# ZhiHuangHn/vtkCloudPoint

Hardware: AMD Instinct MI355X
Metric: Mpoints/s DBSCAN+label @10M pts (higher is better)
Workload: dtype f64; 1 GPU; C4: 10000000-pt cloud (half uniform background, 200 Gaussian blobs), one monolithic DBImproved.dbscan, metric L1_2D, eps 0.1, minPts 10; mode=single, points_total=10000000, points_per_gpu=10000000, clusters=27380, resident_in_hbm=True

## Files before the change

vtkcloudpoint_amd/csrc/dbscan.hip:

```cpp
#include <string.h>

#include <cmath>
#include <cstdlib>
#include <cstring>
#include <limits>
#include <vector>

#include "bounds.hpp"
#include "dbscan_engine.hpp"
#include "grid_common.hpp"

using namespace vcpg;

namespace {

#ifndef VCP_UNR2
#define VCP_UNR2 4
#endif
#ifndef VCP_UNR3
#define VCP_UNR3 2
#endif
#ifndef VCP_UNRW
#define VCP_UNRW 4
#endif
// ... 49 lines not shown
  double q[3], r[3];
  load_exact<GD>(xs, p, q);
  load_exact<GD>(xs, j, r);
  return within<METRIC>(q, r, thr);
}

template <int GD>
struct RowOrder;
template <>
struct RowOrder<2> {
  static constexpr int at(int k) { return k; }
};
template <>
struct RowOrder<3> {
  static constexpr int at(int k) {
    constexpr int o[9] = {1, 3, 4, 5, 7, 0, 2, 6, 8};
    return o[k];
  }
};

template <int GD, bool OWN_FIRST = false, class F>
__device__ __forceinline__ void for_rows(const int* cc, const GridP& g, const CellTab& ct, F&& f) {
  constexpr int NR = GD == 3 ? 9 : 3;
  const int x0 = max(cc[0] - 1, 0), x1 = min(cc[0] + 1, g.D[0] - 1);
  uint32_t rs[NR], re[NR];
#pragma unroll
  for (int r = 0; r < NR; r++) {
    const int y = cc[1] + (r % 3) - 1;
    const int z = GD == 3 ? cc[2] + (r / 3) - 1 : 0;
    const bool ok = y >= 0 && y < g.D[1] && (GD != 3 || (z >= 0 && z < g.D[2]));
    const uint32_t base = ok ? cell_id<GD>(g, 0, y, z) : 0u;
    rs[r] = re[r] = 0u;
    if (ok) ct_range(ct, base + x0, base + x1 + 1, rs[r], re[r]);
  }
  for (int k = 0; k < NR; k++) {
    const int r = OWN_FIRST ? RowOrder<GD>::at(k) : k;
    if (rs[r] < re[r])
      if (!f(rs[r], re[r])) return;
  }
}

template <int GD>
__device__ __forceinline__ void row_bounds(const int* cc, const GridP& g, const CellTab& ct, uint32_t* rs, uint32_t* re) {
  constexpr int NR = GD == 3 ? 9 : 3;
  const int x0 = max(cc[0] - 1, 0), x1 = min(cc[0] + 1, g.D[0] - 1);
#pragma unroll
  for (int r = 0; r < NR; r++) {
    const int y = cc[1] + (r % 3) - 1;
    const int z = GD == 3 ? cc[2] + (r / 3) - 1 : 0;
    const bool ok = y >= 0 && y < g.D[1] && (GD != 3 || (z >= 0 && z < g.D[2]));
    const uint32_t base = ok ? cell_id<GD>(g, 0, y, z) : 0u;
    rs[r] = re[r] = 0u;
    if (ok) ct_range(ct, base + x0, base + x1 + 1, rs[r], re[r]);
  }
}

constexpr unsigned XCHUNK = 8;
constexpr unsigned LCHUNK = 1;
__device__ __forceinline__ int64_t xcd_block(unsigned nblocks) {
  const unsigned b = blockIdx.x;
  const unsigned per = nblocks / (8u * XCHUNK);
  if (b >= per * 8u * XCHUNK) return b;
  const unsigned x = b & 7u, i = b >> 3;
  return (int64_t)((i / per) * 8u + x) * per + (i % per);
}

struct WorkList {
  uint32_t* list;
  const uint32_t* scan;
  uint32_t perblk;
  uint32_t nblk;
};

__device__ __forceinline__ uint32_t wl_fetch(const WorkList& w) {
  const uint32_t total = w.scan[w.nblk] - w.scan[0];
  const uint32_t x = blockIdx.x & 7u, i = blockIdx.x >> 3;
  const uint32_t c = (i / w.perblk) * 8u + x;
  const uint32_t lo = (uint32_t)(((uint64_t)total * c) / (8u * LCHUNK));
  const uint32_t hi = (uint32_t)(((uint64_t)total * (c + 1u)) / (8u * LCHUNK));
  const uint32_t t = lo + (i % w.perblk) * TPB + threadIdx.x;
  if (t >= hi) return NONE;
  return w.list[t];
}

__device__ __forceinline__ void wl_count(bool isE, bool isB, uint32_t blk, uint32_t* __restrict__ cntE,
                                         uint32_t* __restrict__ cntB) {
  __shared__ unsigned wc[2][TPB / 64];
  const unsigned long long mE = __ballot(isE), mB = __ballot(isB);
  if ((threadIdx.x & 63) == 0) {
    wc[0][threadIdx.x >> 6] = (unsigned)__popcll(mE);
    wc[1][threadIdx.x >> 6] = (unsigned)__popcll(mB);
  }
  __syncthreads();
  if (threadIdx.x == 0) {
    unsigned a = 0, b = 0;
    for (int k = 0; k < TPB / 64; k++) {
      a += wc[0][k];
      b += wc[1][k];
    }
    cntE[blk] = a;
    cntB[blk] = b;
  }
}

__global__ __launch_bounds__(TPB) void k_wl_fill(const uint8_t* __restrict__ flags, CellTab ct, const uint32_t* __restrict__ scanE,
                                                const uint32_t* __restrict__ scanB, uint32_t* __restrict__ listE,
// ... 138 lines not shown
        if (jj != (uint32_t)p) lnb[(nrec++) * TPB + threadIdx.x] = jj;
      }
      if (cnt >= min_pts) return false;
    }
    return true;
  });
  if (cnt >= min_pts) nrec = min(nrec, no.core_cap);
  uint8_t fl = live && has_cls ? flags[p] : 0;
  bool isE = false, isB = false;
  if (!live) {
  } else if (cnt >= min_pts) {
    fl |= F_CORE;
    if (!(fl & F_CLASSED)) {
      fl |= F_EXPAND;
      isE = true;
    } else {
      isB = true;
    }
  } else {
    isB = cnt > 1;
  }
  if (isB) fl |= F_BCAND;
  if (live) {
    flags[p] = fl | (uint8_t)(nrec << 4);
    parent[p] = isE ? (uint32_t)p : NONE;
    if (isE) minord[p] = NONE;
  }
  nbr_flush(no, lnb, lnb + no.NB * TPB, nrec, blk, p, live);
  wl_count(isE, isB, (uint32_t)blk, blkE, blkB);
}

template <int GD>
struct CoreTile;
template <>
struct CoreTile<2> {
  static constexpr int NR = 3, CAP = 512;
  union {
    float2 pt[3][512 + 4];
    uint32_t lout[15 * TPB];
  };
  uint32_t lo[3], hi[3];
  __device__ __forceinline__ void put(int r, uint32_t k, const float* __restrict__ s32, uint32_t pos) {
    pt[r][k] = reinterpret_cast<const float2*>(s32)[pos];
  }
  __device__ __forceinline__ void get(int r, uint32_t k, float* c) const {
    const float2 v = pt[r][k];
    c[0] = v.x;
    c[1] = v.y;
  }
};

template <int GD>
__device__ __forceinline__ bool tile_bounds(CoreTile<GD>& t, bool live, const int* cc, const GridP& g,
                                            const CellTab& ct, uint32_t* rs, uint32_t* re) {
  constexpr int NR = CoreTile<GD>::NR;
  if (threadIdx.x < NR) {
    t.lo[threadIdx.x] = NONE;
    t.hi[threadIdx.x] = 0u;
  }
  if (live) {
    row_bounds<GD>(cc, g, ct, rs, re);
  } else {
#pragma unroll
    for (int r = 0; r < NR; r++) rs[r] = re[r] = 0u;
  }
  __syncthreads();
#pragma unroll
  for (int r = 0; r < NR; r++) {
    const unsigned long long m = __ballot(rs[r] < re[r]);
    if (m) {
      const int f = __ffsll((long long)m) - 1, l = 63 - __clzll((long long)m);
      const uint32_t a = (uint32_t)__builtin_amdgcn_readlane((int)rs[r], f);
      const uint32_t b = (uint32_t)__builtin_amdgcn_readlane((int)re[r], l);
      if ((threadIdx.x & 63) == 0) {
        atomicMin(&t.lo[r], a);
        atomicMax(&t.hi[r], b);
      }
    }
  }
  __syncthreads();
  bool fits = true;
#pragma unroll
  for (int r = 0; r < NR; r++) fits = fits && (t.hi[r] <= t.lo[r] || t.hi[r] - t.lo[r] <= (uint32_t)CoreTile<GD>::CAP);
  return fits;
}

template <int GD>
__device__ __forceinline__ void tile_load(CoreTile<GD>& t, const float* __restrict__ sorted32,
                                          int32_t (*tg)[CoreTile<GD>::CAP + 4] = nullptr,
                                          const int32_t* __restrict__ sgroup = nullptr) {
#pragma unroll
  for (int r = 0; r < CoreTile<GD>::NR; r++) {
    const uint32_t lo = t.lo[r], hi = t.hi[r];
    if (hi > lo)
      for (uint32_t k = threadIdx.x; k < hi - lo; k += TPB) {
        t.put(r, k, sorted32, lo + k);
        if (tg) tg[r][k] = sgroup[lo + k];
      }
  }
  __syncthreads();
}

template <int GD, int METRIC>
__device__ __forceinline__ void nbr_flush_masks(const NbrOut& no, uint32_t* lout, const uint32_t* hm, const uint32_t* rs,
                                                const uint32_t* re, bool rescan, int nrec, double thr, const ExactSrc& xs,
                                                int64_t blk, int64_t p, bool live,
                                                const int32_t* __restrict__ sgroup = nullptr) {
  if (no.NB == 0) return;
  constexpr int NR = CoreTile<GD>::NR;
  __shared__ uint32_t wtot[TPB / 64];
  const int lane = threadIdx.x & 63, w = threadIdx.x >> 6;
  uint32_t pre, wsum;
  wave_prefix_small((uint32_t)nrec, pre, wsum);
  if (lane == 0) wtot[w] = wsum;
  __syncthreads();
  uint32_t total = 0;
  for (int k = 0; k < TPB / 64; k++) {
    if (k < w) pre += wtot[k];
    total += wtot[k];
  }
  if (live) no.off[p] = (uint16_t)pre;
  int k = 0;
  if (rescan) {
    double q[3];
    load_exact<GD>(xs, (uint32_t)p, q);
#pragma unroll
    for (int r = 0; r < NR; r++)
      for (uint32_t j = rs[r]; j < re[r] && k < nrec; j++) {
        double rr[3];
        load_exact<GD>(xs, j, rr);
        if (j != (uint32_t)p && within<METRIC>(q, rr, thr) && (!sgroup || sgroup[j] == sgroup[p])) lout[pre + (k++)] = j;
      }
  } else {
#pragma unroll
    for (int r = 0; r < NR; r++) {
      uint32_t m = hm[r];
      while (m != 0u && k < nrec) {
        const uint32_t pos = rs[r] + (uint32_t)(__ffs((int)m) - 1);
        m &= m - 1u;
        if (pos != (uint32_t)p) lout[pre + (k++)] = pos;
      }
    }
  }
  __syncthreads();
  uint32_t* dst = no.nbr + (size_t)blk * (size_t)(no.NB * TPB);
  for (uint32_t i = threadIdx.x; i < total; i += TPB) dst[i] = lout[i];
}

template <int GD, int METRIC, bool GROUPED = false>
__global__ __launch_bounds__(TPB) void k_core_lds(ExactSrc xs, GridP g, double thr, int min_pts,
                                                 CellTab ct, const int32_t* __restrict__ sgroup, uint8_t* __restrict__ flags,
                                                 uint32_t* __restrict__ parent, uint32_t* __restrict__ minord,
                                                 uint32_t* __restrict__ blkE, uint32_t* __restrict__ blkB, NbrOut no,
                                                 const float* __restrict__ sorted32, Screen sc, bool has_cls) {
  constexpr int NR = CoreTile<GD>::NR;
  constexpr int OWN = NR / 2;
  __shared__ CoreTile<GD> t;
  __shared__ int32_t tg[GROUPED ? NR : 1][CoreTile<GD>::CAP + 4];
  const uint32_t nin = *ct.nin;
  const int64_t blk = xcd_block(gridDim.x);
  int64_t p = blk * TPB + threadIdx.x;
  const bool live = p < nin;
  int cc[3] = {0, 0, 0};
  float qf[3] = {0.f, 0.f, 0.f};
  int32_t myg = 0;
  if (live) {
    load_pt32<GD>(sorted32, p, qf);
    cell_of32<GD>(qf, g, cc);
    if (GROUPED) myg = sgroup[p];
  }
  uint32_t rs[NR], re[NR];
  const bool fits = tile_bounds<GD>(t, live, cc, g, ct, rs, re);
  constexpr int UNR = 4;
  const uint32_t scLO = sc.lo < 0.0f ? 0u : __float_as_uint(sc.lo) + 1u;
  const uint32_t scS = __float_as_uint(sc.hi) + 1u - scLO;
  int cnt = 0;
  uint32_t hm[NR], ovf = 0u;
#pragma unroll
  for (int r = 0; r < NR; r++) hm[r] = 0u;
  if (fits) {
    if constexpr (GROUPED) tile_load<GD>(t, sorted32, tg, sgroup);
    else tile_load<GD>(t, sorted32);
    if (live) {
#pragma unroll
      for (int k = 0; k < NR; k++) {
        const int r = RowOrder<GD>::at(k);
        if (cnt >= min_pts || rs[r] >= re[r]) continue;
        const uint32_t lo = t.lo[r];
        const uint32_t e = re[r] - lo, a = rs[r] - lo;
        for (uint32_t j = a; j < e; j += UNR) {
          float c[UNR][3];
#pragma unroll
          for (int u = 0; u < UNR; u++) t.get(r, j + u, c[u]);
          uint32_t w[UNR], nib = 0;
#pragma unroll
          for (int u = UNR - 1; u >= 0; u--) {
            w[u] = __float_as_uint(value32<METRIC>(qf, c[u])) - scLO;
            if (GROUPED) w[u] = tg[r][j + u] == myg ? w[u] : scS;
            nib = __builtin_amdgcn_alignbit(nib, w[u] - scS, 31);
          }
          nib &= 0xFu >> (4u - min(e - j, 4u));
          if (min(min(w[0], w[1]), min(w[2], w[3])) < scS) {
            double q[3];
            load_exact<GD>(xs, (uint32_t)p, q);
#pragma unroll
            for (int u = 0; u < UNR; u++)
              if (((nib >> u) & 1u) && w[u] < scS) {
                double rr[3];
                load_exact<GD>(xs, lo + j + u, rr);
                if (!within<METRIC>(q, rr, thr)) nib &= ~(1u << u);
              }
          }
          cnt += __popc(nib);
          const uint32_t sh = j - a;
          const uint32_t first32 = (uint32_t)((int32_t)(sh - 32u) >> 31);
          hm[r] |= (nib << (sh & 31u)) & first32;
          ovf |= nib & ~first32;
          if (cnt >= min_pts) break;
        }
      }
    }
  } else if (live) {
#pragma unroll
    for (int k = 0; k < NR; k++) {
      const int r = RowOrder<GD>::at(k);
      if (cnt >= min_pts) continue;
      for (uint32_t j = rs[r]; j < re[r]; j += UNR) {
        float rr[UNR][3];
#pragma unroll
        for (int u = 0; u < UNR; u++) load_pt32<GD>(sorted32, min(j + u, re[r] - 1), rr[u]);
        uint32_t nib = 0;
#pragma unroll
        for (int u = 0; u < UNR; u++)
          nib |= ((j + u < re[r]) && (!GROUPED || sgroup[j + u] == myg) &&
                  within_scr<GD, METRIC>(qf, rr[u], sc, xs, (uint32_t)p, j + u, thr)) ? (1u << u) : 0u;
        cnt += __popc(nib);
        const uint32_t sh = j - rs[r];
        hm[r] |= sh < 32u ? nib << sh : 0u;
        ovf |= sh < 32u ? 0u : nib;
        if (cnt >= min_pts) break;
      }
    }
  }
  const bool rescan = live && no.NB > 0 && ovf != 0u && cnt < min_pts;
  int nrec = 0;
  if (live && no.NB > 0) {
    if (rescan) {
      nrec = max(cnt - 1, 0);
    } else {
#pragma unroll
      for (int r = 0; r < NR; r++) nrec += __popc(hm[r]);
      const uint32_t sb = (uint32_t)p - rs[OWN];
      if (rs[OWN] < re[OWN] && sb < 32u && ((hm[OWN] >> sb) & 1u)) nrec--;
    }
    nrec = min(nrec, cnt >= min_pts ? no.core_cap : no.NB);
  }
  uint8_t fl = live && has_cls ? flags[p] : 0;
  bool isE = false, isB = false;
  if (!live) {
  } else if (cnt >= min_pts) {
    fl |= F_CORE;
    if (!(fl & F_CLASSED)) {
      fl |= F_EXPAND;
      isE = true;
    } else {
      isB = true;
    }
  } else {
    isB = cnt > 1;
  }
  if (isB) fl |= F_BCAND;
  if (live) {
    flags[p] = fl | (uint8_t)(nrec << 4);
    parent[p] = isE ? (uint32_t)p : NONE;
    if (isE) minord[p] = NONE;
  }
  nbr_flush_masks<GD, METRIC>(no, t.lout, hm, rs, re, rescan, nrec, thr, xs, blk, p, live, GROUPED ? sgroup : nullptr);
  wl_count(isE, isB, (uint32_t)blk, blkE, blkB);
}

__device__ __forceinline__ uint32_t ld_parent(const uint32_t* parent, uint32_t x) {
  return __hip_atomic_load(&parent[x], __ATOMIC_RELAXED, __HIP_MEMORY_SCOPE_AGENT);
}

__device__ __forceinline__ uint32_t ld_parent_cached(const uint32_t* parent, uint32_t x) {
  return __hip_atomic_load(&parent[x], __ATOMIC_RELAXED, __HIP_MEMORY_SCOPE_WAVEFRONT);
}

__device__ __forceinline__ uint32_t uf_root(uint32_t* parent, uint32_t x) {
  uint32_t p = ld_parent_cached(parent, x);
  while (p != x) {
    const uint32_t gp = ld_parent_cached(parent, p);
    if (gp == p) return p;
    __hip_atomic_store(&parent[x], gp, __ATOMIC_RELAXED, __HIP_MEMORY_SCOPE_WAVEFRONT);
    x = gp;
    p = ld_parent_cached(parent, x);
  }
  return x;
}
// ... 608 lines not shown
double l2_threshold(double eps) {
  if (std::isinf(eps)) return eps;
  double t = eps * eps;
  if (std::isinf(t)) t = std::numeric_limits<double>::max();
  while (std::sqrt(t) > eps) t = std::nextafter(t, 0.0);
  for (;;) {
    double u = std::nextafter(t, std::numeric_limits<double>::infinity());
    if (std::isinf(u) || std::sqrt(u) > eps) break;
    t = u;
  }
  return t;
}

Screen screen_bounds(int metric, int gd, double thr, double E) {
  Screen sc;
  sc.lo = -1.0f;
  sc.hi = INFINITY;
  if (!(thr >= 0.0) || !std::isfinite(E)) return sc;
  if ((thr > 0.0 && thr < 1e-30) || E > 1e18) return sc;
  const double u = 5.9604644775390625e-08;
  const double alpha = 2.0 * u * E * (1.0 + 2.0 * u);
  double err;
  bool lo_ok = true;
  if (metric == VCP_L1_2D) {
    err = 2.0 * alpha * (1.0 + u) + 2.0 * u * (1.0 + u) * thr;
  } else {
    err = 2.0 * alpha * std::sqrt((double)gd * thr) * (1.0 + u) + (double)gd * alpha * alpha + 6.0 * u * (1.0 + u) * thr;
    lo_ok = std::sqrt(thr) > 4.0 * alpha * std::sqrt((double)gd);
  }
  err = err * 1.0625 + 1e-14 * thr + 1e-300;
  const double lo = thr - err, hi = thr + err;
  if (std::isfinite(hi)) {
    float h = (float)hi;
    if ((double)h < hi) h = std::nextafterf(h, INFINITY);
    sc.hi = h;
  }
  if (lo_ok && lo >= 0.0 && std::isfinite(lo)) {
    float l = (float)lo;
    if ((double)l > lo) l = std::nextafterf(l, -INFINITY);
    sc.lo = l;
  } else if (lo_ok && std::isinf(thr) && thr > 0) {
    sc.lo = 3.4028234663852886e38f;
  }
  return sc;
}

unsigned list_perblk(int64_t n) {
  const int64_t band = (n + 8 * LCHUNK - 1) / (8 * LCHUNK) + 1;
  return vcp_blocks(band, TPB);
}

struct Switches {
  int64_t cells_per_point;
  bool screen_off, lists_off, core_global;
  int core_cap, join_all;
};
const Switches& switches() {
  static const Switches sw = [] {
    Switches s;
    const char* e = getenv("VCP_CELL_BUDGET");
    const long v = e ? atol(e) : 32;
    s.cells_per_point = (int64_t)(v < 1 ? 1 : v > 4096 ? 4096 : v);
    s.screen_off = getenv("VCP_NO_SCREEN") != nullptr;
    s.lists_off = getenv("VCP_NO_LISTS") != nullptr;
    s.core_global = getenv("VCP_CORE_GLOBAL") != nullptr;
    s.core_cap = getenv("VCP_CORE_CAP") ? atoi(getenv("VCP_CORE_CAP")) : -1;
    s.join_all = getenv("VCP_JOIN_ALL") ? atoi(getenv("VCP_JOIN_ALL")) : -1;
    return s;
  }();
  return sw;
}

struct EnginePinned {
  double bounds[8];
  uint32_t unclassed;
  uint32_t n_comp;
  unsigned long long counters[CNT_WORDS];
};
static_assert(sizeof(EnginePinned) <= 1024, "the engine's region of vcp_ctx::pinned");
EnginePinned* engine_pinned(vcp_ctx* ctx) { return reinterpret_cast<EnginePinned*>(ctx->pinned); }

struct Call {
  const double* d_coords;
  int64_t n;
  int stride, metric;
  double eps;
  int min_pts;
  int32_t cf_in;
  const uint8_t* d_in_classed;
  int32_t* d_labels;
  uint8_t *d_is_core, *d_is_classed;
  int32_t* cf_out;
  int64_t* dist_evals;
  const DbscanExt* ext;
  int gd = 2;
  unsigned nb = 0;
  const int32_t* d_group = nullptr;
  const uint32_t* d_ord = nullptr;
  uint32_t* d_group_twice = nullptr;
  int G = 0, glo = 0, ghi = 0;
  bool slab = false;
  double* h = nullptr;
  bool all_finite = false;
  double thr = 0.0;
  GridP g;
  Screen sc{-1.0f, INFINITY};
  bool flags_set = false, part_out = false;
  ExactSrc xs{nullptr, nullptr, 0};
  NbrOut no{nullptr, nullptr, 0, 0};
};
void call_derive(Call& c) {
  const DbscanExt* ext = c.ext;
  const bool grouped = ext && ext->d_group;
  c.gd = c.metric == VCP_L2_3D ? 3 : 2;
  c.nb = vcp_blocks(c.n, TPB);
  c.d_group = grouped ? ext->d_group : nullptr;
  c.d_ord = ext ? ext->d_ord : nullptr;
  c.d_group_twice = grouped ? ext->d_group_twice : nullptr;
// ... 245 lines not shown
    return vcp_fail(ctx, VCP_ERR_UNSUPPORTED, "the cloud's extent overflows binary64 (coordinate - origin is infinite)");
  g.scale = 1.0;
  if (Emax > 1e30 || (Emax > 0.0 && Emax < 1e-20)) g.scale = std::ldexp(1.0, -std::ilogb(Emax));
  g.inv_h = std::isinf(cellw) ? 0.0 : 1.0 / (cellw * g.scale);
  g.ncells = (uint32_t)ncells;
  return VCP_OK;
}

int stage_grid_build(vcp_ctx* ctx, Call& c, const Workspace& ws) {
  GridBuildArgs ga;
  ga.d_coords = c.d_coords;
  ga.n = c.n;
  ga.stride = c.stride;
  ga.gd = c.gd;
  ga.g = c.g;
  ga.d_group = c.d_group;
  ga.glo = c.glo;
  ga.ghi = c.ghi;
  ga.d_ord = c.d_ord;
  ga.d_in_classed = c.d_in_classed;
  ga.ctwords = ws.ctwords;
  ga.ctdense = ws.ctdense;
  ga.ctcount = ws.ctcount;
  ga.sidx = c.d_ord ? ws.cellof : nullptr;
  ga.sorted32 = ws.sorted32;
  ga.sord = ws.sord;
  ga.sgroup = ws.sgroup;
  ga.flags = ws.flags;
  ga.pos = c.part_out ? nullptr : ws.pos;
  VCP_TRY(vcp_grid_build_partition(ctx, ga));
  c.xs = ExactSrc{c.d_coords, c.d_ord ? ws.cellof : ws.sord, c.stride};
  return VCP_OK;
}

template <int GD, int METRIC, bool GROUPED>
int stage_core(vcp_ctx* ctx, Call& c, const Workspace& ws, const Switches& sw) {
  hipStream_t st = ctx->stream;
  const int64_t n = c.n;
  const unsigned nb = c.nb;
  vcp_phase(ctx, "core_count");
  NbrOut& no = c.no;
  if (!sw.lists_off && !c.d_in_classed && !c.slab && c.min_pts >= 2 && c.min_pts <= 16) {
    no.NB = c.min_pts - 1;
    VCP_TRY(vcp_ensure(ctx, ctx->b_nbr, (size_t)no.NB * (size_t)nb * TPB * 4));
    VCP_TRY(vcp_ensure(ctx, ctx->b_nboff, (size_t)nb * TPB * 2));
    no.nbr = ctx->b_nbr.as<uint32_t>();
    no.off = ctx->b_nboff.as<uint16_t>();
    no.core_cap = (GD == 2 && (uint64_t)n < (uint64_t)c.g.ncells) ? std::min(no.NB, CORE_LIST) : no.NB;
    if (sw.core_cap >= 0) no.core_cap = std::min(no.NB, sw.core_cap);
  }
  const size_t lds_nb = (size_t)no.NB * TPB * 4;
  bool tiled = false;
  if constexpr (GD == 2) {
    if (!GROUPED || !sw.core_global) {
      VCP_LAUNCH(ctx, (k_core_lds<GD, METRIC, GROUPED>), dim3(nb), dim3(TPB), 0, st, c.xs, c.g, c.thr, c.min_pts, ws.ct,
                      ws.sgroup, ws.flags, ws.parent, ws.minord, ws.blkE, ws.blkB, no, ws.sorted32, c.sc, c.flags_set);
      tiled = true;
    }
  }
  if (!tiled)
    VCP_LAUNCH(ctx, (k_core<GD, METRIC, GROUPED>), dim3(nb), dim3(TPB), 2 * lds_nb, st, c.xs, c.g, c.thr, c.min_pts, ws.ct,
                    ws.sgroup, ws.flags, ws.parent, ws.minord, ws.blkE, ws.blkB, no, ws.sorted32, c.sc, c.flags_set);
  VCP_TRY(vcp_exclusive_scan_u32(ctx, ws.blkE, ws.blkE, 2 * ((int64_t)nb + 2), nullptr));
  VCP_LAUNCH(ctx, k_wl_fill, dim3(nb), dim3(TPB), 0, st, ws.flags, ws.ct, ws.blkE, ws.blkB, ws.wlE.list, ws.wlB.list,
                  ws.seedflag, ws.nw, ws.counters, c.d_group_twice, (uint32_t)(GROUPED ? c.G : 0));
  return VCP_OK;
}

template <int GD, int METRIC, bool GROUPED>
int stage_union(vcp_ctx* ctx, const Call& c, const Workspace& ws, const Switches& sw) {
  hipStream_t st = ctx->stream;
  const int64_t n = c.n;
  const unsigned nb = c.nb, nbl = ws.nbl;
  const GridP& g = c.g;
  const NbrOut& no = c.no;
  vcp_phase(ctx, "union");
  const bool pre = GD == 2 || no.NB > 0;
  if (no.NB > 0) {
    VCP_LAUNCH(ctx, k_union_init_list, dim3(nbl), dim3(TPB), 0, st, ws.flags, ws.parent, no, ws.wlE);
    const bool all = sw.join_all >= 0 ? sw.join_all != 0 : (uint64_t)n >= (uint64_t)g.ncells;
    if (all) VCP_LAUNCH(ctx, k_flatten0<2>, dim3(nbl), dim3(TPB), 0, st, ws.parent, ws.wlE, ws.flags, no);
    else VCP_LAUNCH(ctx, k_flatten0<1>, dim3(nbl), dim3(TPB), 0, st, ws.parent, ws.wlE, ws.flags, no);
    VCP_LAUNCH(ctx, k_flatten0<0>, dim3(nbl), dim3(TPB), 0, st, ws.parent, ws.wlE, ws.flags, no);
  } else if (GD == 2) {
    VCP_LAUNCH(ctx, (k_union_init<GD, METRIC, GROUPED>), dim3(nbl), dim3(TPB), 0, st, c.xs, g, c.thr, ws.ct, ws.sgroup,
                    ws.flags, ws.parent, ws.wlE, ws.sorted32, c.sc);
    VCP_LAUNCH(ctx, k_flatten0<0>, dim3(nbl), dim3(TPB), 0, st, ws.parent, ws.wlE, ws.flags, no);
  }
  const bool dense = pre && (uint64_t)n > (uint64_t)DENSE_PER_CELL * g.ncells;
  if (dense) {
    VCP_TRY(vcp_ensure(ctx, ctx->b_aux0, ((size_t)nb * (TPB / 64) + 2) * 4));
    uint32_t* chunkroot = ctx->b_aux0.as<uint32_t>();
    VCP_LAUNCH(ctx, k_chunkroot, dim3(nb), dim3(TPB), 0, st, ws.parent, ws.ct, chunkroot);
    VCP_LAUNCH(ctx, (k_union<GD, METRIC, GROUPED, true, true>), dim3(nbl), dim3(TPB), 0, st, c.xs, g, c.thr, ws.ct,
                    ws.sgroup, ws.parent, ws.wlE, ws.sorted32, c.sc, chunkroot);
  } else if (pre)
    VCP_LAUNCH(ctx, (k_union<GD, METRIC, GROUPED, true>), dim3(nbl), dim3(TPB), 0, st, c.xs, g, c.thr, ws.ct, ws.sgroup,
                    ws.parent, ws.wlE, ws.sorted32, c.sc);
  else
    VCP_LAUNCH(ctx, (k_union<GD, METRIC, GROUPED, false>), dim3(nbl), dim3(TPB), 0, st, c.xs, g, c.thr, ws.ct, ws.sgroup,
                    ws.parent, ws.wlE, ws.sorted32, c.sc);
  return VCP_OK;
}

int stage_slab_handoff(vcp_ctx* ctx, const Call& c, const Workspace& ws) {
  hipStream_t st = ctx->stream;
  const unsigned nb = c.nb;
// ... 374 lines not shown
```

vtkcloudpoint_amd/csrc/grid_common.hpp:

```cpp
#pragma once
#include "vcp_ctx.hpp"

namespace vcpg {

constexpr int TPB = 256;
constexpr uint8_t F_CORE = 1, F_CLASSED = 2, F_EXPAND = 4, F_BCAND = 8;
constexpr uint32_t NONE = 0xFFFFFFFFu;

constexpr int CNT_LONELY = 0, CNT_MISSING = 0, CNT_SEED_TOTAL = 2, CNT_GROUP_EVALS = 3;
constexpr int CNT_SPREAD = 32;
constexpr int CNT_UNCLASSED = 4, CNT_TWICE = CNT_UNCLASSED + CNT_SPREAD, CNT_WORDS = CNT_TWICE + CNT_SPREAD;

struct GridP {
  double mn[3];
  double inv_h;
  double scale;
  int D[3];
  uint32_t ncells;
};

template <int GD>
__device__ __forceinline__ uint32_t cell_id(const GridP& g, int cx, int cy, int cz) {
  uint32_t id = (uint32_t)cy * (uint32_t)g.D[0] + (uint32_t)cx;
  if (GD == 3) id += (uint32_t)cz * (uint32_t)g.D[0] * (uint32_t)g.D[1];
// ... 38 lines not shown
}

template <int GD>
__device__ __forceinline__ void load_in(const double* __restrict__ c, int64_t i, int stride, double* q) {
  if (GD == 2 && stride == 2) {
    double2 v = *reinterpret_cast<const double2*>(c + 2 * i);
    q[0] = v.x;
    q[1] = v.y;
  } else {
#pragma unroll
    for (int a = 0; a < GD; a++) q[a] = c[i * stride + a];
  }
}

template <int GD>
__device__ __forceinline__ uint32_t cell_of(const double* q, const GridP& g, int* cc) {
  cc[0] = cell_coord(q[0], g.mn[0], g.scale, g.inv_h, g.D[0]);
  cc[1] = cell_coord(q[1], g.mn[1], g.scale, g.inv_h, g.D[1]);
  cc[2] = 0;
  if (GD == 3) cc[2] = cell_coord(q[2], g.mn[2], g.scale, g.inv_h, g.D[2]);
  return cell_id<GD>(g, cc[0], cc[1], cc[2]);
}

template <int GD>
__device__ __forceinline__ uint32_t cell_of32(const float* qf, const GridP& g, int* cc) {
  cc[0] = cell_coord32(qf[0], g.inv_h, g.D[0]);
  cc[1] = cell_coord32(qf[1], g.inv_h, g.D[1]);
  cc[2] = 0;
  if (GD == 3) cc[2] = cell_coord32(qf[2], g.inv_h, g.D[2]);
  return cell_id<GD>(g, cc[0], cc[1], cc[2]);
}

struct CellTab {
  const uint4* words;
  const uint32_t* dense;
  const uint32_t* nin;
};

__device__ __forceinline__ uint32_t ct_start(const CellTab& t, uint32_t cell) {
  const uint4 w = t.words[cell >> 5];
  const uint32_t i = cell & 31u, below = (1u << i) - 1u;
  if ((w.x & w.y & below) == 0u) return w.z + (uint32_t)__popc(w.x & below) + 2u * (uint32_t)__popc(w.y & below);
  return t.dense[(size_t)w.w * 32u + i];
}
__device__ __forceinline__ uint32_t ct_from_word(const CellTab& t, const uint4 w, uint32_t cell) {
  const uint32_t i = cell & 31u, below = (1u << i) - 1u;
  if ((w.x & w.y & below) == 0u) return w.z + (uint32_t)__popc(w.x & below) + 2u * (uint32_t)__popc(w.y & below);
  return t.dense[(size_t)w.w * 32u + i];
}
__device__ __forceinline__ void ct_range(const CellTab& t, uint32_t c0, uint32_t c1, uint32_t& s, uint32_t& e) {
  const uint4 w0 = t.words[c0 >> 5];
  s = ct_from_word(t, w0, c0);
  e = (c1 >> 5) == (c0 >> 5) ? ct_from_word(t, w0, c1) : ct_start(t, c1);
}

struct Screen {
  float lo, hi;
};

template <int GD>
__device__ __forceinline__ void load_pt32(const float* __restrict__ c, int64_t i, float* q) {
  if (GD == 2) {
    const float2 v = *reinterpret_cast<const float2*>(c + 2 * i);
    q[0] = v.x;
    q[1] = v.y;
  } else {
    const float4 v = *reinterpret_cast<const float4*>(c + 4 * i);
    q[0] = v.x;
    q[1] = v.y;
    q[2] = v.z;
  }
}
template <int GD>
__device__ __forceinline__ void store_pt32(float* __restrict__ c, int64_t i, const double* q, const GridP& g) {
  if (GD == 2) {
    *reinterpret_cast<float2*>(c + 2 * i) = make_float2(rel32(q[0], g.mn[0], g.scale), rel32(q[1], g.mn[1], g.scale));
  } else {
    *reinterpret_cast<float4*>(c + 4 * i) =
        make_float4(rel32(q[0], g.mn[0], g.scale), rel32(q[1], g.mn[1], g.scale), rel32(q[2], g.mn[2], g.scale), 0.0f);
  }
}

struct ExactSrc {
  const double* base;
  const uint32_t* idx;
  int stride;
};
template <int GD>
__device__ __forceinline__ void load_exact(const ExactSrc& xs, uint32_t p, double* q) {
  const int64_t i = xs.idx ? (int64_t)xs.idx[p] : (int64_t)p;
  load_in<GD>(xs.base, i, xs.stride, q);
}

}

struct GridBuildArgs {
  const double* d_coords = nullptr;
  int64_t n = 0;
  int stride = 2, gd = 2;
  vcpg::GridP g;
  const int32_t* d_group = nullptr;
  int glo = 0, ghi = 0;
  const uint32_t* d_ord = nullptr;
  const uint8_t* d_in_classed = nullptr;
  uint4* ctwords = nullptr;
  uint32_t* ctdense = nullptr;
// ... 28 lines not shown
```

vtkcloudpoint_amd/csrc/gridbuild.hip:

```cpp
#include <algorithm>
#include <mutex>
#include <unordered_map>

#include "grid_common.hpp"

using namespace vcpg;

namespace {

constexpr int PT = 1024;
constexpr int PCH_MIN = 8192;
constexpr int FT = 1024;
constexpr uint32_t MAXB = 8192;
constexpr uint32_t wcap(int) { return 4096u; }
constexpr uint32_t QUEUE_FROM = 32;

typedef float4 Rec;

template <int GD>
__device__ __forceinline__ Rec rec_make(const float* qf, uint32_t idx, uint32_t cell) {
  return GD == 2 ? make_float4(qf[0], qf[1], __uint_as_float(idx), __uint_as_float(cell))
                 : make_float4(qf[0], qf[1], qf[2], __uint_as_float(idx));
}
template <int GD>
// ... 521 lines not shown
  const uint32_t nq = *qcount;
  for (uint32_t qi = blockIdx.x; qi < nq; qi += gridDim.x) {
    const uint2 q = queue[qi];
    const uint32_t b = q.x, w0 = q.y;
    uint32_t s, e;
    bucket_range(bstart, bstride, total, b, B, s, e);
    const uint32_t m = e - s;
    for (uint32_t j = s + threadIdx.x; j < e; j += FT) {
      const Rec r = rec[j];
      uint32_t i;
      const uint32_t p = ct_start(ct, rec_cell<GD>(r, g, i)) + rk[j] - s - w0;
      if (p < WCAP) stage_put<GD>(s32, sidx, p, r, i);
    }
    __syncthreads();
    fine_flush<GD, GROUPED>(s + w0, min(WCAP, m - w0), s32, sidx, ord, in_classed, group, sorted32, sord, sidx_out, sgroup,
                            flags, pos);
    __syncthreads();
  }
}

constexpr int OT = 1024, OPT = 16;
constexpr int OWT = 512;

template <int OWSH>
__global__ __launch_bounds__(OT) void k_out_scatter(const uint32_t* __restrict__ sord, const uint32_t* __restrict__ labk,
                                                   int64_t n, uint32_t OB, uint32_t* __restrict__ gcur,
                                                   uint2* __restrict__ rec) {
  extern __shared__ uint32_t h[];
  for (uint32_t k = threadIdx.x; k < OB; k += OT) h[k] = 0;
  __syncthreads();
  const int64_t first = (int64_t)blockIdx.x * (OT * OPT);
  uint32_t o[OPT], w[OPT], r[OPT];
#pragma unroll
  for (int k = 0; k < OPT; k++) {
    const int64_t p = first + (int64_t)k * OT + threadIdx.x;
    o[k] = NONE;
    if (p < n) {
      o[k] = sord[p];
      w[k] = labk[p];
      r[k] = atomicAdd(&h[o[k] >> OWSH], 1u);
    }
  }
  __syncthreads();
  for (uint32_t k = threadIdx.x; k < OB; k += OT) {
    const uint32_t c = h[k];
    if (c) h[k] = atomicAdd(&gcur[k], c);
  }
  __syncthreads();
#pragma unroll
  for (int k = 0; k < OPT; k++) {
    if (o[k] == NONE) continue;
    const uint32_t bk = o[k] >> OWSH;
    rec[((size_t)bk << OWSH) + h[bk] + r[k]] = make_uint2(o[k], w[k]);
  }
}

template <int OWSH>
__global__ __launch_bounds__(OWT) void k_out_write(const uint2* __restrict__ rec, int64_t n, bool have_in_classed,
                                                  int32_t cf_in, int32_t* __restrict__ labels,
                                                  uint8_t* __restrict__ is_core, uint8_t* __restrict__ is_classed,
                                                  unsigned long long* __restrict__ counters, uint32_t* __restrict__ gcur) {
  extern __shared__ __attribute__((aligned(16))) uint32_t sw[];
  if (threadIdx.x == 0) gcur[blockIdx.x] = 0u;
  const int64_t lo = (int64_t)blockIdx.x << OWSH;
  const uint32_t cnt = (uint32_t)min((int64_t)1 << OWSH, n - lo);
  unsigned unclassed = 0;
  for (uint32_t j = threadIdx.x; j < cnt; j += OWT) {
    const uint2 v = rec[lo + j];
    sw[v.x - (uint32_t)lo] = v.y;
    if (!(v.y & 2u)) unclassed++;
  }
  __syncthreads();
  auto lab_of = [&](uint32_t w) { return (w >> 2) ? cf_in + (int32_t)(w >> 2) : 0; };
  auto core_of = [](uint32_t w) { return (uint32_t)((w & 3u) == 1u); };
  auto cls_of = [](uint32_t w) { return (uint32_t)((w & 2u) != 0u || (w >> 2) != 0u); };
  const bool vec = (((uintptr_t)labels & 15u) | ((uintptr_t)is_core & 3u) | ((uintptr_t)is_classed & 3u)) == 0;
  const uint32_t c4 = vec ? cnt >> 2 : 0u;
  for (uint32_t j = threadIdx.x; j < c4; j += OWT) {
    const uint4 w = reinterpret_cast<const uint4*>(sw)[j];
    const int4 l = make_int4(lab_of(w.x), lab_of(w.y), lab_of(w.z), lab_of(w.w));
    if (have_in_classed) {
      if (l.x) labels[lo + 4 * j] = l.x;
      if (l.y) labels[lo + 4 * j + 1] = l.y;
      if (l.z) labels[lo + 4 * j + 2] = l.z;
      if (l.w) labels[lo + 4 * j + 3] = l.w;
    } else {
      reinterpret_cast<int4*>(labels + lo)[j] = l;
    }
    if (is_core)
      reinterpret_cast<uint32_t*>(is_core + lo)[j] = core_of(w.x) | core_of(w.y) << 8 | core_of(w.z) << 16 | core_of(w.w) << 24;
    if (is_classed)
      reinterpret_cast<uint32_t*>(is_classed + lo)[j] = cls_of(w.x) | cls_of(w.y) << 8 | cls_of(w.z) << 16 | cls_of(w.w) << 24;
  }
  for (uint32_t j = (c4 << 2) + threadIdx.x; j < cnt; j += OWT) {
    const uint32_t w = sw[j];
    const int32_t l = lab_of(w);
    if (!have_in_classed || l) labels[lo + j] = l;
    if (is_core) is_core[lo + j] = (uint8_t)core_of(w);
    if (is_classed) is_classed[lo + j] = (uint8_t)cls_of(w);
  }
  if (have_in_classed) {
    __shared__ unsigned wc[OWT / 64];
#pragma unroll
    for (int d = 32; d > 0; d >>= 1) unclassed += __shfl_down(unclassed, d, 64);
    if ((threadIdx.x & 63) == 0) wc[threadIdx.x >> 6] = unclassed;
    __syncthreads();
// ... 55 lines not shown
    VCP_TRY(vcp_ensure(ctx, ctx->b_bstart, ((size_t)pg.B + 2) * 4));
    VCP_LAUNCH(ctx, k_part_split<GD>, dim3(pg.NS), dim3(FT), 0, st, rec, ctx->b_rec2.as<Rec>(), counts, total, pg.nchunk,
                    pg.NS, pg.a, pg.csh, pg.B, a.g, ctx->b_bstart.as<uint32_t>());
    rec = ctx->b_rec2.as<Rec>();
    bstart = ctx->b_bstart.as<uint32_t>();
    bstride = 1;
  }
  vcp_phase(ctx, "part_fine");
  VCP_TRY(vcp_ensure(ctx, ctx->b_rank, (size_t)a.n * 4));
  VCP_TRY(vcp_ensure(ctx, ctx->b_bstate, (size_t)pg.B + 16));
  uint8_t* bstate = ctx->b_bstate.as<uint8_t>();
  VCP_LAUNCH(ctx, (k_part_fine_small<GD, GROUPED>), dim3(pg.B), dim3(FS), 0, st, rec, bstart, bstride, total, pg.B, pg.csh,
                  a.g, a.d_ord, a.d_in_classed, a.d_group, a.ctwords, a.ctdense, a.ctcount, bstate, a.sorted32, a.sord,
                  a.sidx, a.sgroup, a.flags, a.pos);
  VCP_LAUNCH(ctx, (k_part_fine<GD, GROUPED>), dim3(pg.B), dim3(FT), lds_f, st, rec, ctx->b_rank.as<uint32_t>(), bstart,
                  bstride, total, pg.B, pg.csh, a.g, a.d_ord, a.d_in_classed, a.d_group, a.ctwords, a.ctdense, a.ctcount,
                  a.sorted32, a.sord, a.sidx, a.sgroup, a.flags, a.pos, queue, qcount, bstate);
  {
    const size_t lds_w = (size_t)wcap(GD) * ((GD == 2 ? 8 : 16) + 4);
    VCP_TRY(allow_lds(ctx, k_part_fine_windows<GD, GROUPED>, lds_w));
    const unsigned gw = (unsigned)std::min<size_t>(768, (size_t)a.n / wcap(GD) + 1);
    const CellTab ct{a.ctwords, a.ctdense, a.ctcount + 1};
    VCP_LAUNCH(ctx, (k_part_fine_windows<GD, GROUPED>), dim3(gw), dim3(FT), lds_w, st, rec, ctx->b_rank.as<uint32_t>(),
                    bstart, bstride, total, pg.B, a.g, a.d_ord, a.d_in_classed, a.d_group, ct, a.sorted32,
                    a.sord, a.sidx, a.sgroup, a.flags, a.pos, queue, qcount);
  }
  return VCP_OK;
}

}

int vcp_grid_build_partition(vcp_ctx* ctx, const GridBuildArgs& a) {
  const bool grouped = a.d_group != nullptr;
  if (a.gd == 3) {
    if (grouped) return vcp_fail(ctx, VCP_ERR_ARG, "grouped calls are 2-D");
    return build<3, false>(ctx, a);
  }
  return grouped ? build<2, true>(ctx, a) : build<2, false>(ctx, a);
}

template <int OWSH>
static int output_partition(vcp_ctx* ctx, const GridOutputArgs& a) {
  hipStream_t st = ctx->stream;
  const uint32_t OB = (uint32_t)((a.n + (1 << OWSH) - 1) >> OWSH);
  const void* before = ctx->b_outcur.p;
  const size_t before_cap = ctx->b_outcur.cap;
  VCP_TRY(vcp_ensure(ctx, ctx->b_outcur, ((size_t)OB + 8) * 4));
  if (ctx->b_outcur.p != before || ctx->b_outcur.cap != before_cap)
    VCP_HIP(ctx, hipMemsetAsync(ctx->b_outcur.p, 0, ctx->b_outcur.cap, st));
  VCP_TRY(vcp_ensure(ctx, ctx->b_rec, (size_t)OB << (OWSH + 3)));
  uint32_t* gcur = ctx->b_outcur.as<uint32_t>();
  uint2* rec = ctx->b_rec.as<uint2>();
  VCP_TRY(allow_lds(ctx, k_out_write<OWSH>, (size_t)4 << OWSH));
  vcp_phase(ctx, "out_scatter");
  VCP_LAUNCH(ctx, k_out_scatter<OWSH>, dim3(vcp_blocks(a.n, OT * OPT)), dim3(OT), (size_t)OB * 4, st, a.sord, a.labk, a.n,
                  OB, gcur, rec);
  vcp_phase(ctx, "out_write");
  VCP_LAUNCH(ctx, k_out_write<OWSH>, dim3(OB), dim3(OWT), (size_t)4 << OWSH, st, rec, a.n, a.have_in_classed, a.cf_in,
                  a.labels, a.is_core, a.is_classed, a.counters, gcur);
  return VCP_OK;
}

int vcp_grid_output_partition(vcp_ctx* ctx, const GridOutputArgs& a) {
  if (a.n > ((int64_t)1 << 27)) return vcp_fail(ctx, VCP_ERR_TOO_LARGE, "more than 2^27 points: use the gather output");
  if (a.n >= ((int64_t)1 << 23)) return output_partition<15>(ctx, a);
  if (a.n >= ((int64_t)1 << 22)) return output_partition<14>(ctx, a);
  return output_partition<13>(ctx, a);
}
```

Measured before the change: 7079 Mpoints/s.

## Skip neighbor scans for isolated points via 5x5 cell-count bitplane prefilter

```diff
diff --git a/vtkcloudpoint_amd/csrc/dbscan.hip b/vtkcloudpoint_amd/csrc/dbscan.hip
--- a/vtkcloudpoint_amd/csrc/dbscan.hip
+++ b/vtkcloudpoint_amd/csrc/dbscan.hip
@@ -125,6 +125,33 @@
     const uint32_t base = ok ? cell_id<GD>(g, 0, y, z) : 0u;
     rs[r] = re[r] = 0u;
     if (ok) ct_range(ct, base + x0, base + x1 + 1, rs[r], re[r]);
+  }
+}
+
+template <int GD>
+__device__ __forceinline__ void row_words(const int* cc, const GridP& g, const CellTab& ct, uint4* w) {
+  static_assert(GD == 2, "three rows");
+  const int x0 = max(cc[0] - 1, 0);
+#pragma unroll
+  for (int r = 0; r < 3; r++) {
+    const int y = cc[1] + r - 1;
+    const bool ok = y >= 0 && y < g.D[1];
+    w[r] = ct.words[(cell_id<GD>(g, 0, ok ? y : cc[1], 0) + (uint32_t)x0) >> 5];
+  }
+}
+template <int GD>
+__device__ __forceinline__ void row_bounds_from(const int* cc, const GridP& g, const CellTab& ct, const uint4* w,
+                                                uint32_t* rs, uint32_t* re) {
+  const int x0 = max(cc[0] - 1, 0), x1 = min(cc[0] + 1, g.D[0] - 1);
+#pragma unroll
+  for (int r = 0; r < 3; r++) {
+    const int y = cc[1] + r - 1;
+    rs[r] = re[r] = 0u;
+    if (y >= 0 && y < g.D[1]) {
+      const uint32_t c0 = cell_id<GD>(g, 0, y, 0) + (uint32_t)x0, c1 = cell_id<GD>(g, 0, y, 0) + (uint32_t)x1 + 1u;
+      rs[r] = ct_from_word(ct, w[r], c0);
+      re[r] = (c1 >> 5) == (c0 >> 5) ? ct_from_word(ct, w[r], c1) : ct_start(ct, c1);
+    }
   }
 }
 
@@ -369,14 +396,19 @@
 
 template <int GD>
 __device__ __forceinline__ bool tile_bounds(CoreTile<GD>& t, bool live, const int* cc, const GridP& g,
-                                            const CellTab& ct, uint32_t* rs, uint32_t* re) {
+                                            const CellTab& ct, uint32_t* rs, uint32_t* re, const uint4* pre = nullptr) {
   constexpr int NR = CoreTile<GD>::NR;
   if (threadIdx.x < NR) {
     t.lo[threadIdx.x] = NONE;
     t.hi[threadIdx.x] = 0u;
   }
   if (live) {
-    row_bounds<GD>(cc, g, ct, rs, re);
+    if constexpr (GD == 2) {
+      if (pre) row_bounds_from<GD>(cc, g, ct, pre, rs, re);
+      else row_bounds<GD>(cc, g, ct, rs, re);
+    } else {
+      row_bounds<GD>(cc, g, ct, rs, re);
+    }
   } else {
 #pragma unroll
     for (int r = 0; r < NR; r++) rs[r] = re[r] = 0u;
@@ -464,7 +496,44 @@
   for (uint32_t i = threadIdx.x; i < total; i += TPB) dst[i] = lout[i];
 }
 
-template <int GD, int METRIC, bool GROUPED = false>
+__device__ __forceinline__ bool quiet_point(bool live, const int* cc, const GridP& g, const CellTab& ct, int min_pts) {
+  const int x0 = max(cc[0] - 2, 0), x1 = min(cc[0] + 2, g.D[0] - 1);
+  constexpr int DY[5] = {0, -1, 1, -2, 2};
+  uint2 w0[5], w1[5];
+  uint32_t c0[5], full[5];
+#pragma unroll
+  for (int k = 0; k < 5; k++) {
+    const int y = cc[1] + DY[k];
+    const bool ok = y >= 0 && y < g.D[1];
+    const uint32_t base = (uint32_t)(ok ? y : cc[1]) * (uint32_t)g.D[0];
+    c0[k] = base + (uint32_t)x0;
+    full[k] = ok ? (2u << (x1 - x0)) - 1u : 0u;
+    w0[k] = ct_planes(ct, c0[k]);
+    w1[k] = ct_planes(ct, base + (uint32_t)x1);
+  }
+  bool sat = false, cand = live;
+  int S = (int)ct_pop_planes(w0[0], w1[0], c0[0], full[0], sat);
+  cand = cand && S < min_pts;
+  if (__ballot(cand) == 0ull) return false;
+  S += (int)(ct_pop_planes(w0[1], w1[1], c0[1], full[1], sat) + ct_pop_planes(w0[2], w1[2], c0[2], full[2], sat));
+  cand = cand && S < min_pts;
+  if (__ballot(cand) == 0ull) return false;
+  S += (int)(ct_pop_planes(w0[3], w1[3], c0[3], full[3], sat) + ct_pop_planes(w0[4], w1[4], c0[4], full[4], sat));
+  cand = cand && S < min_pts;
+  if (cand && sat) {
+    S = 0;
+    for (int dy = -2; dy <= 2; dy++) {
+      const int y = cc[1] + dy;
+      if (y < 0 || y >= g.D[1]) continue;
+      const uint32_t base = (uint32_t)y * (uint32_t)g.D[0];
+      S += (int)ct_pop_exact(ct, base + (uint32_t)x0, base + (uint32_t)x1);
+    }
+    cand = S < min_pts;
+  }
+  return cand;
+}
+
+template <int GD, int METRIC, bool GROUPED = false, bool QUIET = false>
 __global__ __launch_bounds__(TPB) void k_core_lds(ExactSrc xs, GridP g, double thr, int min_pts,
                                                  CellTab ct, const int32_t* __restrict__ sgroup, uint8_t* __restrict__ flags,
                                                  uint32_t* __restrict__ parent, uint32_t* __restrict__ minord,
@@ -481,13 +550,43 @@
   int cc[3] = {0, 0, 0};
   float qf[3] = {0.f, 0.f, 0.f};
   int32_t myg = 0;
+  uint32_t cid = 0u;
   if (live) {
     load_pt32<GD>(sorted32, p, qf);
-    cell_of32<GD>(qf, g, cc);
+    cid = cell_of32<GD>(qf, g, cc);
     if (GROUPED) myg = sgroup[p];
   }
+  bool act = live;
   uint32_t rs[NR], re[NR];
-  const bool fits = tile_bounds<GD>(t, live, cc, g, ct, rs, re);
+  bool fits;
+  if constexpr (QUIET) {
+    const unsigned long long lm = __ballot(live);
+    bool sparse = false;
+    if (lm != 0ull) {
+      const uint32_t c_first = (uint32_t)__builtin_amdgcn_readlane((int)cid, __ffsll((long long)lm) - 1);
+      const uint32_t c_last = (uint32_t)__builtin_amdgcn_readlane((int)cid, 63 - __clzll((long long)lm));
+      sparse = c_last - c_first >= (uint32_t)__popcll(lm);
+    }
+    uint4 rw[3];
+    row_words<GD>(cc, g, ct, rw);
+    if (sparse) act = live && !quiet_point(live, cc, g, ct, min_pts);
+    fits = tile_bounds<GD>(t, act, cc, g, ct, rs, re, rw);
+  } else {
+    fits = tile_bounds<GD>(t, act, cc, g, ct, rs, re);
+  }
+  if constexpr (QUIET) {
+    bool none = true;
+#pragma unroll
+    for (int r = 0; r < NR; r++) none = none && t.hi[r] <= t.lo[r];
+    if (none) {
+      if (live) {
+        flags[p] = has_cls ? (uint8_t)(flags[p] & F_CLASSED) : (uint8_t)0;
+        parent[p] = NONE;
+      }
+      if (threadIdx.x == 0) blkE[blk] = blkB[blk] = 0u;
+      return;
+    }
+  }
   constexpr int UNR = 4;
   const uint32_t scLO = sc.lo < 0.0f ? 0u : __float_as_uint(sc.lo) + 1u;
   const uint32_t scS = __float_as_uint(sc.hi) + 1u - scLO;
@@ -498,7 +597,7 @@
   if (fits) {
     if constexpr (GROUPED) tile_load<GD>(t, sorted32, tg, sgroup);
     else tile_load<GD>(t, sorted32);
-    if (live) {
+    if (act) {
 #pragma unroll
       for (int k = 0; k < NR; k++) {
         const int r = RowOrder<GD>::at(k);
@@ -537,7 +636,7 @@
         }
       }
     }
-  } else if (live) {
+  } else if (act) {
 #pragma unroll
     for (int k = 0; k < NR; k++) {
       const int r = RowOrder<GD>::at(k);
@@ -559,9 +658,9 @@
       }
     }
   }
-  const bool rescan = live && no.NB > 0 && ovf != 0u && cnt < min_pts;
+  const bool rescan = act && no.NB > 0 && ovf != 0u && cnt < min_pts;
   int nrec = 0;
-  if (live && no.NB > 0) {
+  if (act && no.NB > 0) {
     if (rescan) {
       nrec = max(cnt - 1, 0);
     } else {
@@ -1276,7 +1375,7 @@
 
 struct Switches {
   int64_t cells_per_point;
-  bool screen_off, lists_off, core_global;
+  bool screen_off, lists_off, core_global, no_quiet;
   int core_cap, join_all;
 };
 const Switches& switches() {
@@ -1288,6 +1387,7 @@
     s.screen_off = getenv("VCP_NO_SCREEN") != nullptr;
     s.lists_off = getenv("VCP_NO_LISTS") != nullptr;
     s.core_global = getenv("VCP_CORE_GLOBAL") != nullptr;
+    s.no_quiet = getenv("VCP_NO_QUIET") != nullptr;
     s.core_cap = getenv("VCP_CORE_CAP") ? atoi(getenv("VCP_CORE_CAP")) : -1;
     s.join_all = getenv("VCP_JOIN_ALL") ? atoi(getenv("VCP_JOIN_ALL")) : -1;
     return s;
@@ -1639,7 +1739,15 @@
   const size_t lds_nb = (size_t)no.NB * TPB * 4;
   bool tiled = false;
   if constexpr (GD == 2) {
-    if (!GROUPED || !sw.core_global) {
+    const bool quiet = !GROUPED && !sw.no_quiet && !c.d_in_classed && !c.slab && c.min_pts >= 2 &&
+                       (uint64_t)n < (uint64_t)c.g.ncells;
+    if (quiet) {
+      if constexpr (!GROUPED)
+        VCP_LAUNCH(ctx, (k_core_lds<GD, METRIC, false, true>), dim3(nb), dim3(TPB), 0, st, c.xs, c.g, c.thr, c.min_pts,
+                        ws.ct, ws.sgroup, ws.flags, ws.parent, ws.minord, ws.blkE, ws.blkB, no, ws.sorted32, c.sc,
+                        c.flags_set);
+      tiled = true;
+    } else if (!GROUPED || !sw.core_global) {
       VCP_LAUNCH(ctx, (k_core_lds<GD, METRIC, GROUPED>), dim3(nb), dim3(TPB), 0, st, c.xs, c.g, c.thr, c.min_pts, ws.ct,
                       ws.sgroup, ws.flags, ws.parent, ws.minord, ws.blkE, ws.blkB, no, ws.sorted32, c.sc, c.flags_set);
       tiled = true;
diff --git a/vtkcloudpoint_amd/csrc/grid_common.hpp b/vtkcloudpoint_amd/csrc/grid_common.hpp
--- a/vtkcloudpoint_amd/csrc/grid_common.hpp
+++ b/vtkcloudpoint_amd/csrc/grid_common.hpp
@@ -114,6 +114,22 @@
   const uint4 w0 = t.words[c0 >> 5];
   s = ct_from_word(t, w0, c0);
   e = (c1 >> 5) == (c0 >> 5) ? ct_from_word(t, w0, c1) : ct_start(t, c1);
+}
+
+__device__ __forceinline__ uint2 ct_planes(const CellTab& t, uint32_t cell) {
+  return *reinterpret_cast<const uint2*>(&t.words[cell >> 5]);
+}
+__device__ __forceinline__ uint32_t ct_pop_planes(const uint2 w0, const uint2 w1, uint32_t c0, uint32_t full, bool& sat) {
+  const unsigned long long m = (unsigned long long)full << (c0 & 31u);
+  const uint32_t m0 = (uint32_t)m, m1 = (uint32_t)(m >> 32);
+  const uint32_t l0 = w0.x & m0, h0 = w0.y & m0, l1 = w1.x & m1, h1 = w1.y & m1;
+  sat = sat || ((l0 & h0) | (l1 & h1)) != 0u;
+  return (uint32_t)(__popc(l0) + __popc(l1)) + 2u * (uint32_t)(__popc(h0) + __popc(h1));
+}
+__device__ __forceinline__ uint32_t ct_pop_exact(const CellTab& t, uint32_t c0, uint32_t c1) {
+  uint32_t s, e;
+  ct_range(t, c0, c1 + 1u, s, e);
+  return e - s;
 }
 
 struct Screen {
```

Result: no change. 7229 Mpoints/s, median of 6 (+2.1%).

## Stage output scatter records in LDS to coalesce bucketed global writes

Applied to the files above, without the earlier changes.

```diff
diff --git a/vtkcloudpoint_amd/csrc/gridbuild.hip b/vtkcloudpoint_amd/csrc/gridbuild.hip
--- a/vtkcloudpoint_amd/csrc/gridbuild.hip
+++ b/vtkcloudpoint_amd/csrc/gridbuild.hip
@@ -597,6 +597,72 @@
     if (o[k] == NONE) continue;
     const uint32_t bk = o[k] >> OWSH;
     rec[((size_t)bk << OWSH) + h[bk] + r[k]] = make_uint2(o[k], w[k]);
+  }
+}
+
+template <int OWSH, int PER>
+__global__ __launch_bounds__(OT) void k_out_scatter_staged(const uint32_t* __restrict__ sord,
+                                                          const uint32_t* __restrict__ labk, int64_t n, uint32_t OB,
+                                                          uint32_t* __restrict__ gcur, uint2* __restrict__ rec) {
+  constexpr uint32_t T = OT * PER;
+  extern __shared__ __attribute__((aligned(16))) uint32_t sm[];
+  uint2* tile = reinterpret_cast<uint2*>(sm);
+  uint32_t* h = sm + 2 * T;
+  uint32_t* delta = h + OB;
+  __shared__ uint32_t wsum[OT / 64];
+  for (uint32_t k = threadIdx.x; k < OB; k += OT) h[k] = 0;
+  __syncthreads();
+  const int64_t first = (int64_t)blockIdx.x * T;
+  uint32_t o[PER], w[PER], r[PER];
+#pragma unroll
+  for (int k = 0; k < PER; k++) {
+    const int64_t p = first + (int64_t)k * OT + threadIdx.x;
+    const int64_t pc = min(p, n - 1);
+    o[k] = sord[pc];
+    w[k] = labk[pc];
+    if (p >= n) o[k] = NONE;
+  }
+#pragma unroll
+  for (int k = 0; k < PER; k++)
+    if (o[k] != NONE) r[k] = atomicAdd(&h[o[k] >> OWSH], 1u);
+  __syncthreads();
+  for (uint32_t k = threadIdx.x; k < OB; k += OT) {
+    const uint32_t c = h[k];
+    if (c) delta[k] = atomicAdd(&gcur[k], c);
+  }
+  const uint32_t per = (OB + OT - 1) / OT, k0 = threadIdx.x * per, k1 = min(k0 + per, OB);
+  uint32_t loc = 0;
+  for (uint32_t k = k0; k < k1; k++) loc += h[k];
+  uint32_t inc = loc;
+  const int lane = threadIdx.x & 63, wv = threadIdx.x >> 6;
+#pragma unroll
+  for (int d = 1; d < 64; d <<= 1) {
+    const uint32_t t = __shfl_up(inc, d, 64);
+    if (lane >= d) inc += t;
+  }
+  if (lane == 63) wsum[wv] = inc;
+  __syncthreads();
+  uint32_t pre = inc - loc;
+  for (int k = 0; k < wv; k++) pre += wsum[k];
+  for (uint32_t k = k0; k < k1; k++) {
+    const uint32_t c = h[k];
+    h[k] = pre;
+    delta[k] = (k << OWSH) + delta[k] - pre;
+    pre += c;
+  }
+  __syncthreads();
+#pragma unroll
+  for (int k = 0; k < PER; k++)
+    if (o[k] != NONE) tile[h[o[k] >> OWSH] + r[k]] = make_uint2(o[k], w[k]);
+  __syncthreads();
+  const uint32_t m = (uint32_t)min((int64_t)T, n - first);
+#pragma unroll
+  for (int k = 0; k < PER; k++) {
+    const uint32_t s = (uint32_t)k * OT + threadIdx.x;
+    if (s < m) {
+      const uint2 v = tile[s];
+      rec[delta[v.x >> OWSH] + s] = v;
+    }
   }
 }
 
@@ -758,9 +824,25 @@
   uint32_t* gcur = ctx->b_outcur.as<uint32_t>();
   uint2* rec = ctx->b_rec.as<uint2>();
   VCP_TRY(allow_lds(ctx, k_out_write<OWSH>, (size_t)4 << OWSH));
+  static const int stage = env_int("VCP_OUT_STAGE", 3, 0, 3);
+  constexpr size_t LDS_CU = 160 * 1024 - 64;
+  auto lds_staged = [&](int per) { return (size_t)OT * per * 8 + (size_t)OB * 8; };
+  int per = stage == 0 ? 0 : stage == 1 || (stage == 3 && OB <= 512) ? OPT / 2 : OPT;
+  if (per == OPT && lds_staged(OPT) > LDS_CU) per = OPT / 2;
+  if (per == OPT / 2 && lds_staged(OPT / 2) > LDS_CU) per = 0;
+  if (per == OPT) VCP_TRY(allow_lds(ctx, (k_out_scatter_staged<OWSH, OPT>), lds_staged(OPT)));
+  if (per == OPT / 2) VCP_TRY(allow_lds(ctx, (k_out_scatter_staged<OWSH, OPT / 2>), lds_staged(OPT / 2)));
   vcp_phase(ctx, "out_scatter");
-  VCP_LAUNCH(ctx, k_out_scatter<OWSH>, dim3(vcp_blocks(a.n, OT * OPT)), dim3(OT), (size_t)OB * 4, st, a.sord, a.labk, a.n,
-                  OB, gcur, rec);
+  if (per == OPT) {
+    VCP_LAUNCH(ctx, (k_out_scatter_staged<OWSH, OPT>), dim3(vcp_blocks(a.n, OT * OPT)), dim3(OT), lds_staged(OPT), st,
+                    a.sord, a.labk, a.n, OB, gcur, rec);
+  } else if (per == OPT / 2) {
+    VCP_LAUNCH(ctx, (k_out_scatter_staged<OWSH, OPT / 2>), dim3(vcp_blocks(a.n, OT * OPT / 2)), dim3(OT),
+                    lds_staged(OPT / 2), st, a.sord, a.labk, a.n, OB, gcur, rec);
+  } else {
+    VCP_LAUNCH(ctx, k_out_scatter<OWSH>, dim3(vcp_blocks(a.n, OT * OPT)), dim3(OT), (size_t)OB * 4, st, a.sord, a.labk,
+                    a.n, OB, gcur, rec);
+  }
   vcp_phase(ctx, "out_write");
   VCP_LAUNCH(ctx, k_out_write<OWSH>, dim3(OB), dim3(OWT), (size_t)4 << OWSH, st, rec, a.n, a.have_in_classed, a.cf_in,
                   a.labels, a.is_core, a.is_classed, a.counters, gcur);
@@ -769,6 +851,7 @@
 
 int vcp_grid_output_partition(vcp_ctx* ctx, const GridOutputArgs& a) {
   if (a.n > ((int64_t)1 << 27)) return vcp_fail(ctx, VCP_ERR_TOO_LARGE, "more than 2^27 points: use the gather output");
+  if (a.n <= 0) return VCP_OK;
   if (a.n >= ((int64_t)1 << 23)) return output_partition<15>(ctx, a);
   if (a.n >= ((int64_t)1 << 22)) return output_partition<14>(ctx, a);
   return output_partition<13>(ctx, a);
```

Result: faster. 7058 Mpoints/s before, 7282 Mpoints/s after, median of 6 (+3.2%).
